# krejciadam/hammock

Hardware: AMD Instinct MI355X
Metric: pairwise BLOSUM62 ShiftedScorer scores/sec (all-vs-all, thresholded neighbour list) (higher is better)
Workload: dtype u8 (8-bit SWAR lanes, host-proven ranges with 16-bit / literal fallbacks; scores are int32-exact)

## Files before the change

### hammock_amd/csrc/hmk_common.cpp

```cpp
#include <atomic>

#include "hmk_ctx.h"
#include "hmk_grid.h"

namespace hmk {

static std::atomic<int> g_test_grid_cap{0};
void set_test_grid_cap(int cap) { g_test_grid_cap.store(cap < 1 ? 0 : cap, std::memory_order_relaxed); }
uint32_t capped_grid(const char *kernel, uint32_t wanted) {
    const int cap = g_test_grid_cap.load(std::memory_order_relaxed);
    if (cap < 1 || wanted <= (uint32_t)cap) return wanted;
    std::fprintf(stderr, "[hmk grid] %s %u -> %d\n", kernel, wanted, cap);
    return (uint32_t)cap;
}

namespace impl {

thread_local std::string g_last_error;

void Switches::read() {
    auto flag = [](const char *name) { return getenv(name) != nullptr; };
    auto num = [](const char *name, int dflt) { const char *v = getenv(name); return v ? atoi(v) : dflt; };
    *this = Switches();
    greedy_timing = flag("HMK_GREEDY_TIMING");
    no_band = flag("HMK_NO_BAND");
    no_rows_kernel = flag("HMK_NO_ROWS_KERNEL");
    key_sort = flag("HMK_NO_KEY_SORT") ? 0 : num("HMK_KEY_SORT_KEYS", 2) == 1 ? 1 : 2;
    no_row_shared = flag("HMK_NO_ROW_SHARED");
    adj_8byte = flag("HMK_ADJ_8BYTE");
    local_literal = flag("HMK_LOCAL_LITERAL");
    local_signed = flag("HMK_LOCAL_SIGNED");
    local_no_pk = flag("HMK_LOCAL_NO_PK");
    multi_replicate = flag("HMK_MULTI_REPLICATE");
    multi_force_copies = flag("HMK_MULTI_FORCE_COPIES");
    if (const char *v = getenv("HMK_SECOND_LOOP")) second_loop = std::strcmp(v, "device") == 0 ? 1 : 2;
    phase1_threads = std::max(0, num("HMK_PHASE1_THREADS", 0));
    phase1_window = std::max(0, num("HMK_PHASE1_WINDOW", 0));
    if (const char *v = getenv("HMK_PHASE1_HOST_BAND")) {
        host_band_rows = std::max(0, atoi(v));
        if (const char *c = std::strchr(v, ',')) host_band_far_t = std::max(0, atoi(c + 1));
    }
    loop_chain = getenv("HMK_LOOP_CHAIN") ? (num("HMK_LOOP_CHAIN", 0) != 0 ? 1 : 0) : -1;
    loop_passes = std::min(8, std::max(0, num("HMK_LOOP_PASSES", 0)));
// ... 218 lines not shown
```

### hammock_amd/csrc/hmk_ctx.h

```cpp
#ifndef HMK_CTX_H
#define HMK_CTX_H
#include <hip/hip_runtime_api.h>

#include <algorithm>
#include <chrono>
#include <condition_variable>
#include <functional>
#include <future>
#include <memory>
#include <cstdio>
#include <cstdlib>
#include <cstring>
#include <map>
#include <mutex>
#include <numeric>
#include <string>
#include <tuple>
#include <thread>
#include <vector>

#include "hmk_internal.h"
#include "hmk_kernels.h"
#include "hmk_sizing.h"

// ... 54 lines not shown
    SB_MERGE_CNT, SB_MERGE_OSTART, SB_MERGE_SCR, SB_MERGE_SCAN,
    SB_LINK_TAB, SB_LINK_OUT,
    SB_SPLIT_SCORES,
    SB_CC_PARENT, SB_CC_SIZE,
    SB_CC_STATE, SB_CC_RUNS,
    SB_ALIGN_SLOT, SB_ALIGN_MEMB,
    SB_N
};

struct Switches {
    bool greedy_timing = false;
    bool no_band = false;
    bool no_rows_kernel = false;
    int key_sort = 2;
    bool no_row_shared = false;
    bool adj_8byte = false;
    bool local_literal = false;
    bool local_signed = false;
    bool local_no_pk = false;
    bool multi_replicate = false;
    bool multi_force_copies = false;
    int second_loop = 0;
    int phase1_threads = 0, phase1_window = 0;
    int host_band_rows = 0, host_band_far_t = 0;
    int loop_chain = -1;
    int loop_passes = 0;
    int precheck = 0;
    int late_buffers_delay_ms = 0;
    int csr_bucket_shift = 0;
    uint64_t edge_guess = 0;
// ... 9 lines not shown
    Tile *d_tiles = nullptr;
};

struct Plan : PlanArrays {
    bool valid = false;
    int X = 0, p = 0, thr = 0;
    uint32_t part = 0, n_parts = 1;
    uint32_t band_rows = 0;
    int64_t band_req = 0;
    int lbmax = 12, lpad = 16;
    bool exact = false;
    bool rows_exact = false;
    bool no_rows_kernel = false;
    int key_sort = 2;
    bool row_shared = true;
    uint32_t *d_keyrun = nullptr;
    uint32_t *d_keytab = nullptr;
    uint32_t cols_per_tile = 16384;
    uint8_t *d_mb = nullptr;
    std::vector<Group> groups;
    hmk_neighbor_stats stats{};
    uint64_t band_pairs = 0;
    uint32_t q0 = 0, q1 = 0, r0 = 0, r1 = 0;
};

struct PlanLocal : PlanArrays {
    bool valid = false;
    uint32_t part = 0, n_parts = 1;
    uint32_t n_tiles = 0;
    uint64_t pairs = 0;
// ... 261 lines not shown
```

### hammock_amd/csrc/hmk_internal.h

```cpp
#ifndef HMK_INTERNAL_H
#define HMK_INTERNAL_H

#include <stdint.h>

#include <functional>
#include <string>
#include <vector>

#include "../../include/hammock_hip.h"

namespace hmk {


enum { PATH_U8 = 0, PATH_U16 = 1, PATH_DIRECT = 2, PATH_ROWS = 3 };

struct TileClass {
    uint8_t la, lb;
    uint8_t nd;
    uint8_t case_b;
    uint8_t x;
    uint8_t path;
    uint8_t nw;
    uint8_t pad;
    int32_t g;
// ... 19 lines not shown
    uint64_t *edges;
    unsigned long long *counts;
    uint64_t cap_per_shard;
    uint32_t n_tiles;
    uint32_t lpad;
    uint32_t symmetric;
    uint32_t row_is_m;
    uint32_t perm_identity;
    uint32_t *deg;
    uint32_t deg_m_offset;
    const uint32_t *keyrun;
    const uint32_t *keytab;
};

constexpr int KEYTAB_DWORDS = 16;
constexpr bool rows_keyed(int x, int d, int cap, bool exact, int g) { return exact && d == 0 && g == 1 && x == 3 && cap == 12; }
constexpr int rows_key_pos(int x, int l, int q) { return l / 2 - 1 + q < x ? x : l / 2 - 1 + q; }

struct Nbr {
    uint32_t m;
    int32_t s;
    uint32_t id() const { return m; }
    int32_t score() const { return s; }
};
struct NbrPacked {
    uint32_t v;
    uint32_t id() const { return v >> 8; }
    int32_t score() const { return (int32_t)(v & 0xFFu); }
};

struct GreedyCand { int32_t c, mn, covered; };
// ... 84 lines not shown
```

### hammock_amd/csrc/hmk_kernels.h

```cpp
#ifndef HMK_KERNELS_H
#define HMK_KERNELS_H

#include <hip/hip_runtime_api.h>
#include <stdint.h>

#include "hmk_internal.h"

namespace hmk {

int swar_rows_per_tile(int lbmax, int nw, bool exact);
int swar_lbmax_for(int lb);

hipError_t launch_neighbors_swar(int lbmax, int nw, bool exact, const NeighborParams &P,
                                 uint32_t tile_base, uint32_t n_tiles, hipStream_t s);
bool rows_kernel_available(int X, int la, int lb, bool exact);
int rows_cap_for(int lb);
int rows_per_tile_rows(int X, int d, int cap, bool exact);
hipError_t launch_neighbors_rows(int X, int d, int cap, bool exact, const NeighborParams &P, uint32_t tile_base,
                                 uint32_t n_tiles, hipStream_t s);
hipError_t warm_neighbors_rows_module();
hipError_t launch_rows_keytab(const uint8_t *res_sorted, uint32_t lpad, uint32_t n, const uint8_t *mb, int case_b, int X, int L,
                              const uint32_t (&cinit)[8], uint32_t *keytab, uint32_t n_groups);
hipError_t launch_neighbors_direct(const NeighborParams &P, uint32_t tile_base, uint32_t n_tiles,
                                   const int32_t *d_matrix, int max_shift, int shift_penalty, int threshold,
                                   hipStream_t s);
hipError_t launch_probe_spin(unsigned long long *when, long long ticks, hipStream_t s);
hipError_t launch_pairs(int scorer, const uint8_t *res32, const uint8_t *len, const int32_t *d_matrix,
                        const uint32_t *pi, const uint32_t *pj, uint64_t n_pairs, uint32_t r0, uint32_t c0,
                        uint32_t width, int a, int b, int32_t *out, int32_t *out_shift, hipStream_t s);

hipError_t launch_neighbors_local(int lbmax, bool enc, bool force_signed, bool force_unpacked, const NeighborParams &P, uint32_t tile_base,
                                  uint32_t n_tiles, const int32_t *d_matrix, int gap_open, int gap_extend, int threshold, hipStream_t s);

hipError_t launch_neighbors_local_literal(const NeighborParams &P, uint32_t tile_base, uint32_t n_tiles, const int32_t *d_matrix,
// ... 96 lines not shown
```

### hammock_amd/csrc/hmk_pass.cpp

```cpp
#include "hmk_ctx.h"

namespace hmk { namespace impl {

static int make_side_streams(hmk_ctx *ctx) {
    constexpr int n_side = hmk_ctx::N_SIDE, MAX_TRIES = 12;
    unsigned long long *when = nullptr;
    HIPCHK(ctx, hipHostMalloc((void **)&when, 64, hipHostMallocDefault));
    auto side_by_side = [&](hipStream_t a, hipStream_t b, bool *yes) -> hipError_t {
        std::memset(when, 0, 64);
        hipError_t e = launch_probe_spin(when, 6000, a);
        if (e == hipSuccess) e = launch_probe_spin(when + 2, 6000, b);
        if (e == hipSuccess) e = hipStreamSynchronize(a);
        if (e == hipSuccess) e = hipStreamSynchronize(b);
        *yes = when[2] < when[1] && when[0] < when[3];
        return e;
    };
    std::vector<hipStream_t> kept, dropped;
    hipError_t e = hipSuccess;
    for (int t = 0; t < MAX_TRIES && (int)kept.size() < n_side && e == hipSuccess; t++) {
        hipStream_t s = nullptr;
        e = hipStreamCreateWithFlags(&s, hipStreamNonBlocking);
        if (e != hipSuccess) break;
        bool ok = true;
        for (size_t k = 0; k < kept.size() && ok && e == hipSuccess; k++) e = side_by_side(kept[k], s, &ok);
// ... 56 lines not shown
    std::vector<const Group *> order;
    for (const Group &g : pl.groups) order.push_back(&g);
    std::stable_sort(order.begin(), order.end(), [](const Group *a, const Group *b) { return a->work > b->work; });
    uint64_t load[hmk_ctx::N_SIDE] = {0};
    for (const Group *gp : order) {
        const Group &g = *gp;
        int least = 0;
        for (int k = 1; k < n_side; k++) if (load[k] < load[least]) least = k;
        load[least] += g.work;
        hipStream_t s = fork ? sides[least] : stream;
        const uint32_t t0 = which == LAUNCH_REST ? g.base + g.band : g.base;
        const uint32_t cnt = which == LAUNCH_ALL ? g.count : which == LAUNCH_BAND ? g.band : g.count - g.band;
        if (g.path == PATH_DIRECT)
            HIPCHK(ctx, launch_neighbors_direct(P, t0, cnt, ctx->d_M.as<int32_t>(), X, p, thr, s));
        else if (g.path == PATH_ROWS)
            HIPCHK(ctx, launch_neighbors_rows(X, g.nw, g.lbk, pl.rows_exact, P, t0, cnt, s));
        else
            HIPCHK(ctx, launch_neighbors_swar(g.lbk, g.nw, pl.exact, P, t0, cnt, s));
    }
    if (fork)
        for (int k = 0; k < n_side; k++) {
            HIPCHK(ctx, hipEventRecord(ctx->ev_join[k], sides[k]));
            HIPCHK(ctx, hipStreamWaitEvent(stream, ctx->ev_join[k], 0));
        }
    return HMK_OK;
}

bool local_enc(const hmk_ctx *ctx, int gap_open, int gap_extend) {
    return ctx->min_m >= -31 && ctx->max_m <= 31 && gap_open >= -31 && gap_extend >= -31 && gap_open <= 0 && gap_extend <= 0;
}

// ... 165 lines not shown
```

### hammock_amd/csrc/hmk_plan.cpp

```cpp
#include "hmk_ctx.h"

namespace hmk { namespace impl {

template <class T, class Cmp>
void parallel_stable_sort(std::vector<T> &v, Cmp before) {
    const size_t n = v.size();
    const unsigned hw = usable_cpus();
    size_t runs = 1;
    while (runs < 8 && runs < (hw ? hw : 1u) && n / (2 * runs) >= 32768) runs *= 2;
    if (runs == 1) { std::stable_sort(v.begin(), v.end(), before); return; }
    std::vector<size_t> cut(runs + 1);
    for (size_t r = 0; r <= runs; r++) cut[r] = n * r / runs;
    {
        std::vector<std::thread> pool;
        for (size_t r = 1; r < runs; r++) pool.emplace_back([&, r] { std::stable_sort(v.begin() + (long)cut[r], v.begin() + (long)cut[r + 1], before); });
        std::stable_sort(v.begin(), v.begin() + (long)cut[1], before);
        for (std::thread &th : pool) th.join();
    }
    std::vector<T> other(n);
    std::vector<T> *from = &v, *to = &other;
    for (size_t width = 1; width < runs; width *= 2) {
        std::vector<std::thread> pool;
        for (size_t r = 0; r < runs; r += 2 * width) {
            auto job = [&, r] {
// ... 20 lines not shown
    for (int side = 0; side < 2; side++) {
        uint32_t *b = bucket[side];
        std::fill(b, b + HMK_MAX_LEN + 2, 0u);
        for (uint32_t k = lo[side]; k < hi[side]; k++) b[ctx->len[k] + 1]++;
        b[0] = side ? a1 - a0 : 0u;
        for (int l = 0; l <= HMK_MAX_LEN; l++) b[l + 1] += b[l];
        Buckets fill;
        std::memcpy(fill, b, sizeof(fill));
        for (uint32_t k = lo[side]; k < hi[side]; k++) perm[fill[ctx->len[k]]++] = k;
    }
}

using GroupKey = std::tuple<int, int, int>;
struct KernelChoice { bool rows; int lbk; uint32_t R; GroupKey key; };

KernelChoice choose_kernel(const TileClass &tc, int X, bool use_rows, bool rows_exact, bool exact) {
    const int la = tc.la, lb = tc.lb;
    KernelChoice k;
    k.rows = use_rows && tc.path == PATH_U8 && la >= lb && (rows_exact || rows_kernel_available(X, la, lb, false));
    k.lbk = k.rows ? (rows_exact ? lb : rows_cap_for(lb)) : exact ? 12 : swar_lbmax_for(lb);
    k.R = k.rows ? (uint32_t)rows_per_tile_rows(X, la - lb, k.lbk, rows_exact)
                 : tc.path == PATH_DIRECT ? 16u : (uint32_t)swar_rows_per_tile(k.lbk, tc.nw, exact);
    k.key = k.rows ? GroupKey((int)PATH_ROWS, la - lb, k.lbk)
                   : GroupKey((int)tc.path, tc.path == PATH_DIRECT ? 0 : (int)tc.nw, tc.path == PATH_DIRECT ? 0 : k.lbk);
    return k;
}

uint32_t add_class(std::vector<TileClass> &classes, hmk_neighbor_stats &S, const TileClass &tc, bool rows) {
    classes.push_back(tc);
    if (tc.path == PATH_U8) S.classes_u8++;
    else if (tc.path == PATH_U16) S.classes_u16++;
    else S.classes_direct++;
    if (rows) S.classes_rows++;
    return (uint32_t)classes.size() - 1;
}

// ... 190 lines not shown
        c.path = u16 ? PATH_U16 : PATH_U8;
        c.g = (int32_t)g;
        const int lpd = u16 ? 2 : 4, bits = u16 ? 16 : 8;
        const int ndw = (nd + lpd - 1) / lpd;
        c.nw = (uint8_t)ndw;
        for (int t = 0; t < nd; t++) c.cinit[t / lpd] |= (uint32_t)ci[t] << ((t % lpd) * bits);
    }
    *out = c;
}

int build_plan(hmk_ctx *ctx, int X, int p, int thr, uint32_t part, uint32_t n_parts, int64_t band_rows, bool key_sort_ok) {
    Plan &pl = ctx->plan;
    const int want_keys = key_sort_ok ? ctx->sw.key_sort : 0;
    if (pl.valid && pl.X == X && pl.p == p && pl.thr == thr && pl.part == part && pl.n_parts == n_parts &&
        (band_rows < 0 || pl.band_req == band_rows) && pl.no_rows_kernel == ctx->sw.no_rows_kernel && pl.key_sort == want_keys &&
        pl.row_shared == !ctx->sw.no_row_shared)
        return HMK_OK;
    free_plan(pl);
    if (band_rows < 0) band_rows = 0;
    const int64_t band_req = band_rows;
    const bool plan_timing = ctx->sw.greedy_timing;
    const auto plan_t0 = std::chrono::steady_clock::now();
    auto plan_lap = [&](const char *what) {
        if (plan_timing)
            fprintf(stderr, "[hmk plan] %s at %.2f ms\n", what,
                    std::chrono::duration<double, std::milli>(std::chrono::steady_clock::now() - plan_t0).count());
    };
    const uint32_t n = ctx->n;
    if (n == 0) return fail(ctx, HMK_ERR_NO_SEQUENCES, "no sequences set (hmk_set_sequences)");
    if (X < 0) return fail(ctx, HMK_ERR_BAD_ARG, "max_shift must be >= 0");
    if (n_parts == 0 || part >= n_parts) return fail(ctx, HMK_ERR_BAD_ARG, "part must be < n_parts");
// ... 74 lines not shown
    pl.no_rows_kernel = ctx->sw.no_rows_kernel;
    pl.exact = false;
    pl.rows_exact = false;
    if (use_rows && ctx->min_len == ctx->max_len) {
        TileClass t1;
        classify(ctx, ctx->min_len, ctx->min_len, X, p, thr, &t1);
        pl.rows_exact = (t1.path == PATH_U8 || (refine && all_rows_fit)) && rows_kernel_available(X, ctx->min_len, ctx->min_len, true);
    }
    if (!use_rows && ctx->min_len == 12 && ctx->max_len == 12 && X == 3) {
        TileClass t12;
        classify(ctx, 12, 12, X, p, thr, &t12);
        pl.exact = t12.path == PATH_U8 && t12.nw == 2;
    }
    pl.key_sort = want_keys;
    pl.row_shared = !ctx->sw.no_row_shared;
    std::vector<uint32_t> keyrun;
    const int L1 = ctx->min_len;
    const bool key_sorted = pl.key_sort > 0 && pl.rows_exact && !(refine && !all_rows_fit) &&
                            rows_keyed(X, 0, L1, true, rows_per_tile_rows(X, 0, L1, true) / 8) && n >= 2;
    if (key_sorted) {
        const int k0 = rows_key_pos(X, L1, 0), k1 = rows_key_pos(X, L1, 1);
        auto key_of = [&](uint32_t k) { return (uint32_t)ctx->res[ctx->off[k] + k0] * HMK_ALPHABET + ctx->res[ctx->off[k] + k1]; };
        const uint32_t b0 = band_end[L1], b1 = bucket[L1 + 1];
        std::vector<uint32_t> cnt(HMK_ALPHABET * HMK_ALPHABET + 1, 0u), sorted(perm.begin() + b0, perm.begin() + b1);
        for (uint32_t q = b0; q < b1; q++) cnt[key_of(perm[q]) + 1]++;
        for (int v = 0; v < HMK_ALPHABET * HMK_ALPHABET; v++) cnt[v + 1] += cnt[v];
        for (uint32_t q = b0; q < b1; q++) sorted[cnt[key_of(perm[q])]++] = perm[q];
        std::copy(sorted.begin(), sorted.end(), perm.begin() + b0);
        keyrun.resize(2 * (size_t)n);
        uint32_t r0 = 0, r01 = 0;
        for (uint32_t q = 0; q < n; q++) {
            const uint32_t k = perm[q], c0 = ctx->res[ctx->off[k] + k0], c1 = ctx->res[ctx->off[k] + k1];
            if (q > 0) {
                const uint32_t kp = perm[q - 1];
                const bool same0 = ctx->res[ctx->off[kp] + k0] == c0;
                r0 += same0 ? 0u : 1u;
                r01 += (pl.key_sort == 2 && same0 && ctx->res[ctx->off[kp] + k1] == c1) ? 0u : 1u;
            }
            keyrun[2 * (size_t)q] = r0 << 5 | c0;
            keyrun[2 * (size_t)q + 1] = r01 << 5 | c1;
        }
    }
    const uint64_t tile_rows = pl.rows_exact ? (uint64_t)rows_per_tile_rows(X, 0, ctx->min_len, true) : use_rows ? 16 : 6;
    const uint64_t row_groups = (uint64_t)n / tile_rows / n_parts + 1;
    pl.cols_per_tile = 65536;
    while (pl.cols_per_tile > 16384 && row_groups * ((uint64_t)n / (2 * pl.cols_per_tile) + 1) < 8 * 1792)
        pl.cols_per_tile /= 2;
    while (pl.cols_per_tile > 4096 && ((uint64_t)n / tile_rows + 1) * ((uint64_t)n / (2 * pl.cols_per_tile) + 1) < 4096)
        pl.cols_per_tile /= 2;

    std::vector<TileClass> classes;
    std::map<GroupKey, std::vector<Tile>> grouped;
    hmk_neighbor_stats &S = pl.stats;
    S = hmk_neighbor_stats{};
    S.symmetric = ctx->symmetric;
    uint64_t row_chunk_counter = 0;
    for (int la = 1; la <= HMK_MAX_LEN; la++) {
        const uint32_t rb = bucket[la], re = bucket[la + 1];
        if (rb == re) continue;
        for (int lb = 1; lb <= HMK_MAX_LEN; lb++) {
            const uint32_t cb = bucket[lb], ce = bucket[lb + 1];
            if (cb == ce) continue;
// ... 10 lines not shown
                if (refine && tc0.path != PATH_U8 && limit >= 0) {
                    const uint32_t lim = (uint32_t)std::min<long long>(limit, BCAP - 1);
                    split = all_rows_fit ? re
                                         : (uint32_t)(std::upper_bound(bound_sorted.begin() + rb, bound_sorted.begin() + re, lim) -
                                                      bound_sorted.begin());
                    if (split > rb) {
                        TileClass t8;
                        classify(ctx, la, lb, X, p, thr, &t8, lim);
                        if (t8.path == PATH_U8) ranges.push_back(Range{rb, split, t8});
                        else split = rb;
                    }
                }
                if (split < re) ranges.push_back(Range{split, re, tc0});
            }
            for (const Range &rg : ranges) {
                const KernelChoice k = choose_kernel(rg.tc, X, use_rows, pl.rows_exact, pl.exact);
                const uint32_t cls = add_class(classes, S, rg.tc, k.rows);
                std::vector<Tile> &dst = grouped[k.key];
                const bool tri = same && ctx->symmetric;
                for (uint32_t r0 = rg.lo; r0 < rg.hi; r0 += k.R) {
                    if ((row_chunk_counter++ % n_parts) != part) continue;
                    Band band{r0 < band_end[la], band_end[lb], 0};
                    S.pairs_scored += emit_tiles(dst, cls, r0, std::min(k.R, rg.hi - r0), tri ? r0 + 1 : cb, ce, pl.cols_per_tile, true,
                                                 tri ? 1u : same ? 2u : 0u, &band);
                    pl.band_pairs += band.pairs;
                }
            }
        }
    }
    plan_lap("classes and tiles");
    std::vector<Tile> tiles = order_groups(grouped, classes, X, pl.groups);
// ... 194 lines not shown
```

### hammock_amd/csrc/k_neighbors_rows.h

```cpp
#ifndef HMK_NEIGHBORS_ROWS_H
#define HMK_NEIGHBORS_ROWS_H
#include "hmk_device.h"

namespace hmk {

constexpr int ROWS_STAGE_CAPFORM = 320, ROWS_STAGE_EXACT = 640, ROWS_STAGE_SHORT = 1024;
constexpr int ROWS_INLOOP_MAXCELLS = 45;
constexpr int rows_cells(int x, int cap) { return cap * (2 * x + 1) - x * (x + 1); }
constexpr bool rows_inloop(int x, int cap) { return rows_cells(x, cap) > ROWS_INLOOP_MAXCELLS; }
constexpr bool rows_inloop_shape(int x, int d, int cap, bool exact) { return (exact && d > 0) || rows_inloop(x, cap); }
constexpr int rows_stage(int x, int d, int cap, bool exact) {
    return !exact ? ROWS_STAGE_CAPFORM : rows_inloop_shape(x, d, cap, exact) ? ROWS_STAGE_EXACT : ROWS_STAGE_SHORT;
}
constexpr int rows_groups(int x, int , int cap, bool exact) {
    return !exact ? 2 : rows_inloop(x, cap) ? 1 : 2;
}
constexpr bool rows_two_ended(int x, int d, int cap, bool exact, int g) { return exact && !rows_inloop_shape(x, d, cap, exact) && g == 2; }

template <typename T>
__device__ __forceinline__ T rows_table_read(uint32_t addr) {
    return *reinterpret_cast<const volatile HMK_LDS T *>((uintptr_t)addr);
}
constexpr int rows_waves(int nd, int cap, int lds_bytes, bool exact) {
    const int v = cap + 2 * nd + 36 + (exact ? 0 : 6);
// ... 475 lines not shown
#undef HMK_FLUSH_ST
#undef HMK_FLUSH_ST_00
#undef HMK_FLUSH_ST_01
#undef HMK_FLUSH_ST_10
#undef HMK_FLUSH_ST_11
    asm volatile("" ::: "memory");
    drain_end();
    }
}

template <class F, int... Is>
__device__ __forceinline__ void rows_for_each_group(std::integer_sequence<int, Is...>, F &&f) {
    (f(std::integral_constant<int, Is>{}), ...);
}

template <int X, int D, int CAP, bool EXACT_LB, int G, int MODE>
__device__ __forceinline__ void rows_tile(const NeighborParams &P, const uint32_t tile_base, uint8_t *smem) {
    using S = RowsShape<X, D, CAP, EXACT_LB, G>;
    constexpr int ND = S::ND, NI = S::NI, NEND = S::NEND, TAB_BYTES = S::TAB_BYTES;
    constexpr int R = 8 * G;
    constexpr int STAGE_CAP = rows_stage(X, D, CAP, EXACT_LB);
    constexpr int LDS_BYTES = TAB_BYTES + 576 + R * 32 + 4 * STAGE_CAP * 4;
    static_assert(LDS_BYTES == rows_lds_bytes(X, D, CAP, EXACT_LB, G), "rows_lds_bytes must match the LDS map");
    uint8_t *tab = smem;
    uint8_t *mb = smem + TAB_BYTES;
    uint8_t *rowres = mb + 576;
    uint32_t *stage_all = reinterpret_cast<uint32_t *>(rowres + R * 32);

    const Tile T = P.tiles[tile_base + blockIdx.x];
    const TileClass *Cp = P.classes + T.cls;
    const int la = Cp->la;
    int lbs = EXACT_LB ? CAP : (int)Cp->lb;
    const bool case_b = Cp->case_b != 0;
    const int tid = threadIdx.x;
    HMK_LDS uint32_t *stage = (HMK_LDS uint32_t *)stage_all + __builtin_amdgcn_readfirstlane(tid >> 6) * STAGE_CAP;

    constexpr bool KEYED = rows_keyed(X, D, CAP, EXACT_LB, G);
    const bool keyed = KEYED && P.keyrun != nullptr;
    const bool row_shared = keyed && (T.row_shared & 1u) != 0;

    build_begin();
    const uint32_t tab_addr = lds_addr(tab);
    for (int e = tid; e < 576; e += 256) mb[e] = P.mb[e];
    for (int e = tid; e < R * 32; e += 256) {
        const int r = e >> 5, k = e & 31;
        uint8_t v = 0;
        if ((uint32_t)r < T.nrows && (uint32_t)k < P.lpad) v = P.res_sorted[(size_t)(T.row0 + r) * P.lpad + k];
        rowres[e] = v;
    }
    __syncthreads();
    for (int e = tid; e < G * (NI + NEND) * 24 * 2; e += 256) {
        const int h = e & 1, ic = e >> 1;
        const int gi = ic / 24, c = ic - gi * 24;
        const int g = gi / (NI + NEND), k = gi - g * (NI + NEND);
        int i = k < NI ? k : la - 1 - (k - NI);
        const int dst = k < NI ? S::pos_addr(g, k) : S::end_addr(g, k - NI);
        if constexpr (KEYED)
            if (row_shared && k == S::key_pos(0) && h == 1) i = S::key_pos(1);
        uint32_t v = 0;
        if (i >= 0 && i < la) {
#pragma unroll
            for (int q = 0; q < 4; q++) {
                const int r = 8 * g + 4 * h + q;
                if ((uint32_t)r < T.nrows) {
                    const int a = rowres[r * 32 + i];
                    v |= (uint32_t)(case_b ? mb[c * 24 + a] : mb[a * 24 + c]) << (q * 8);
                }
            }
        }
        *reinterpret_cast<uint32_t *>(tab + dst + c * 8 + h * 4) = v;
    }
    __syncthreads();
    build_end();
// ... 8 lines not shown
    const uint32_t col_end = T.col0 + T.ncols;
    const uint32_t n_batches = (T.ncols + 255) / 256;
    const bool interior = T.diag == 0 && T.ncols % 256 == 0;
    const bool prio = true;

    const uint8_t *const res_sorted = P.res_sorted;
    const uint32_t lpad_s = P.lpad;

    constexpr bool INLOOP = rows_inloop_shape(X, D, CAP, EXACT_LB);
    constexpr bool DEFER = EXACT_LB && !INLOOP;
    const uint64_t ka64 = (uint64_t)(uintptr_t)__builtin_amdgcn_kernarg_segment_ptr();
    const uint32_t ka_lo = (uint32_t)ka64, ka_hi = (uint32_t)(ka64 >> 32);
    uint32_t acc[G];
#pragma unroll
    for (int g = 0; g < G; g++) acc[g] = 0;
    static_assert(!KEYED || (G == 1 && 2 * ND <= KEYTAB_DWORDS), "key table entry; one row group per tile");
    static_assert(!KEYED || (S::body_reads(3, false) == 58 && S::body_reads(1, false) == 65 && S::body_reads(0, false) == 72), "ordinary bodies");
    static_assert(!KEYED || (S::body_reads(3, true) == 54 && S::body_reads(1, true) == 60 && S::body_reads(0, true) == 66), "row-shared bodies");
    const uint32_t wave = __builtin_amdgcn_readfirstlane(tid >> 6);
    const uint32_t *kt_tile = nullptr, *kr_wave = nullptr;
    if (keyed) {
        kt_tile = P.keytab + (size_t)(T.row0 >> 3) * (2 * 24 * KEYTAB_DWORDS);
        kr_wave = P.keyrun + 2 * (size_t)(T.col0 + wave * 64);
    }
    auto key_entry = [](const uint32_t *e, uint32_t (&k0)[ND], uint32_t (&k1)[ND]) {
#pragma unroll
        for (int u = 0; u + 1 < ND; u += 2) {
            const u32x4 a = rows_const_load<u32x4>(e + 2 * u);
            k0[u] = a.x; k1[u] = a.y; k0[u + 1] = a.z; k1[u + 1] = a.w;
        }
        if constexpr (ND & 1) {
// ... 14 lines not shown
                const uint32_t last = min(63u, col_end - 1u - wc0);
                ra = rows_const_load<u32x2>(kr_wave);
                const u32x2 rb = rows_const_load<u32x2>(kr_wave + 2 * last);
                if (ra.x == rb.x) kmode = ra.y == rb.y ? 3 : 1;
            }
        }
        uint32_t off[CAP], toff[S::NT];
        S::offsets_of(words, tw, tab_addr, tab_addr, off, toff);
        const bool look = !DEFER || (bt & 3u) == 3u || bt + 1 == n_batches;

        auto one_group = [&](auto gt) {
            constexpr int g = decltype(gt)::value;
            if ((uint32_t)(8 * g) >= T.nrows) return;
            uint32_t W0[ND], W1[ND];
            if constexpr (KEYED) {
                uint32_t ks0[ND], ks1[ND];
                if (kmode == 3) {
                    uint32_t kb0[ND], kb1[ND];
                    key_entry(kt_tile + (ra.x & 31u) * KEYTAB_DWORDS, ks0, ks1);
                    key_entry(kt_tile + (24 + (ra.y & 31u)) * KEYTAB_DWORDS, kb0, kb1);
#pragma unroll
                    for (int u = 0; u < ND; u++) { ks0[u] += kb0[u]; ks1[u] += kb1[u]; }
                    read_phase_begin(prio);
                    if (row_shared) S::template accumulate<g, 3, true>(off, toff, lbs, ks0, ks1, W0, W1);
                    else S::template accumulate<g, 3>(off, toff, lbs, ks0, ks1, W0, W1);
                } else if (kmode == 1) {
                    key_entry(kt_tile + (ra.x & 31u) * KEYTAB_DWORDS, ks0, ks1);
#pragma unroll
                    for (int u = 0; u < ND; u++) asm volatile("" : "+s"(ks0[u]), "+s"(ks1[u]));
                    read_phase_begin(prio);
                    if (row_shared) S::template accumulate<g, 1, true>(off, toff, lbs, ks0, ks1, W0, W1);
                    else S::template accumulate<g, 1>(off, toff, lbs, ks0, ks1, W0, W1);
                } else {
                    read_phase_begin(prio);
                    if (row_shared) S::template accumulate<g, 0, true>(off, toff, lbs, ci, ci, W0, W1);
                    else S::template accumulate<g>(off, toff, lbs, ci, ci, W0, W1);
                }
            } else {
                read_phase_begin(prio);
                S::template accumulate<g>(off, toff, lbs, ci, ci, W0, W1);
            }
            read_phase_end(prio);
// ... 82 lines not shown
    return m;
}
constexpr int rows_lens_waves(int x, int d, int capb) {
    const int lds = rows_lens_lds(x, d, capb);
    int w = rows_waves(2 * x + d + 1, capb, lds, false);
    for (int lb = rows_lens_first(capb); lb <= capb; lb++)
        if (rows_lens_has(x, d, capb, lb) && rows_waves(2 * x + d + 1, lb, lds, true) < w) w = rows_waves(2 * x + d + 1, lb, lds, true);
    return w;
}
template <int X, int D, int CAPB, int MODE, int LB>
__device__ __forceinline__ void rows_lens_pick(const NeighborParams &P, const uint32_t tile_base, uint8_t *smem, int lb) {
    if constexpr (LB > CAPB) {
        rows_tile<X, D, CAPB, false, 2, MODE>(P, tile_base, smem);
    } else {
        if constexpr (rows_lens_has(X, D, CAPB, LB)) {
            if (lb == LB) { rows_tile<X, D, LB, true, 2, MODE>(P, tile_base, smem); return; }
        }
        rows_lens_pick<X, D, CAPB, MODE, LB + 1>(P, tile_base, smem, lb);
    }
}
template <int X, int D, int CAPB, int MODE>
__global__ void __launch_bounds__(256, rows_lens_waves(X, D, CAPB))
k_neighbors_rows_lens(const NeighborParams P, const uint32_t tile_base) {
    __shared__ __attribute__((aligned(16))) uint8_t smem[rows_lens_lds(X, D, CAPB)];
    const int lb = (int)P.classes[P.tiles[tile_base + blockIdx.x].cls].lb;
    rows_lens_pick<X, D, CAPB, MODE, rows_lens_first(CAPB)>(P, tile_base, smem, lb);
}


}
#endif
// ... 1 lines not shown
```

### hammock_amd/csrc/k_neighbors_rows.hip

```cpp
#include "k_rows_shapes.h"

namespace hmk {

int rows_cap_for(int lb) { return lb <= 12 ? 12 : lb <= 16 ? 16 : lb <= 20 ? 20 : 0; }

namespace {
int rows_part_of(int X, int d, int cap, bool exact) {
    if (exact) {
#define HMK_F(PV, XV, L) if (X == XV && d == 0 && cap == L) return PV;
        HMK_ROWS_EXACT_LIST(HMK_F)
#undef HMK_F
        return -1;
    }
#define HMK_C(PV, XV, DV, CAPV) if (X == XV && d == DV && cap == CAPV) return PV;
    HMK_ROWS_CAP_LIST(HMK_C)
#undef HMK_C
    return -1;
}
}

int rows_per_tile_rows(int X, int d, int cap, bool exact) {
    if (rows_part_of(X, d, cap, exact) < 0) return 0;
    return 8 * rows_groups(X, d, cap, exact);
}

bool rows_kernel_available(int X, int la, int lb, bool exact) {
    if (la < lb || lb < 2 * X || X < 1) return false;
    return rows_part_of(X, la - lb, exact ? lb : rows_cap_for(lb), exact) >= 0;
}

hipError_t launch_neighbors_rows(int X, int d, int cap, bool exact, const NeighborParams &P, uint32_t tile_base,
                                 uint32_t n_tiles, hipStream_t s) {
    if (n_tiles == 0) return hipSuccess;
    switch (rows_part_of(X, d, cap, exact)) {
#define HMK_P(p) case p: return launch_rows_part_##p(X, d, cap, exact, P, tile_base, n_tiles, s);
        HMK_P(0) HMK_P(1) HMK_P(2) HMK_P(3) HMK_P(4) HMK_P(5) HMK_P(6) HMK_P(7) HMK_P(8) HMK_P(9) HMK_P(10) HMK_P(11) HMK_P(12)
#undef HMK_P
    }
    return hipErrorInvalidValue;
}

hipError_t warm_neighbors_rows_module() { return warm_rows_part_0(); }

struct KeytabInit { uint32_t w[8]; };
__global__ void __launch_bounds__(256) k_rows_keytab(const uint8_t *__restrict__ res_sorted, uint32_t lpad, uint32_t n,
                                                     const uint8_t *__restrict__ mb, int case_b, int X, int L, const KeytabInit cinit,
                                                     uint32_t *__restrict__ keytab, uint32_t n_groups) {
    const uint64_t e = (uint64_t)blockIdx.x * 256 + threadIdx.x;
    if (e >= (uint64_t)n_groups * 2 * HMK_ALPHABET * KEYTAB_DWORDS) return;
    const int d = (int)(e % KEYTAB_DWORDS), c = (int)(e / KEYTAB_DWORDS % HMK_ALPHABET), q = (int)(e / (KEYTAB_DWORDS * HMK_ALPHABET) % 2);
// ... 29 lines not shown
```

### hammock_amd/csrc/k_rows_part.hip

```cpp
#include "k_rows_shapes.h"

#ifndef HMK_ROWS_PART
#error "compile with -DHMK_ROWS_PART=<part>"
#endif

namespace hmk {

namespace {
template <bool MINE, int X, int D, int CAP, bool EXACT_LB>
struct RowsLaunch {
    static hipError_t go(const NeighborParams &, uint32_t, uint32_t, hipStream_t) { return hipErrorInvalidValue; }
};
template <int X, int D, int CAP, bool EXACT_LB>
struct RowsLaunch<true, X, D, CAP, EXACT_LB> {
    static hipError_t go(const NeighborParams &P, uint32_t tile_base, uint32_t n_tiles, hipStream_t s) {
        return launch_rows_t<X, D, CAP, EXACT_LB>(P, tile_base, n_tiles, s);
    }
};
}

#define HMK_CAT2(a, b) a##b
#define HMK_CAT(a, b) HMK_CAT2(a, b)

hipError_t HMK_CAT(launch_rows_part_, HMK_ROWS_PART)(int X, int d, int cap, bool exact, const NeighborParams &P, uint32_t tile_base,
                                                     uint32_t n_tiles, hipStream_t s) {
    if (exact) {
#define HMK_F(PV, XV, L) \
    if (PV == HMK_ROWS_PART && X == XV && d == 0 && cap == L) return RowsLaunch<PV == HMK_ROWS_PART, XV, 0, L, true>::go(P, tile_base, n_tiles, s);
        HMK_ROWS_EXACT_LIST(HMK_F)
#undef HMK_F
        return hipErrorInvalidValue;
    }
#define HMK_C(PV, XV, DV, CAPV) \
    if (PV == HMK_ROWS_PART && X == XV && d == DV && cap == CAPV) return RowsLaunch<PV == HMK_ROWS_PART, XV, DV, CAPV, false>::go(P, tile_base, n_tiles, s);
    HMK_ROWS_CAP_LIST(HMK_C)
#undef HMK_C
    return hipErrorInvalidValue;
}

#if HMK_ROWS_PART == 0
hipError_t warm_rows_part_0() {
    hipFuncAttributes a;
    return hipFuncGetAttributes(&a, reinterpret_cast<const void *>(&k_neighbors_rows<3, 0, 12, true, rows_groups(3, 0, 12, true), EDGES_PLAIN>));
}
#endif

}
```

### hammock_amd/csrc/k_rows_shapes.h

```cpp
#ifndef HMK_ROWS_SHAPES_H
#define HMK_ROWS_SHAPES_H
#include "k_neighbors_rows.h"

namespace hmk {

template <int X, int D, int CAP, bool EXACT_LB>
static hipError_t launch_rows_t(const NeighborParams &P, uint32_t tile_base, uint32_t n_tiles, hipStream_t s) {
    constexpr int G = rows_groups(X, D, CAP, EXACT_LB);
    if constexpr (!EXACT_LB && (X == 2 || X == 3)) {
        static_assert(G == 2, "the planner gives the capacity groups 16 rows per tile");
        if (P.deg) hipLaunchKernelGGL((k_neighbors_rows_lens<X, D, CAP, EDGES_COUNT>), dim3(n_tiles), dim3(256), 0, s, P, tile_base);
        else hipLaunchKernelGGL((k_neighbors_rows_lens<X, D, CAP, EDGES_PLAIN>), dim3(n_tiles), dim3(256), 0, s, P, tile_base);
        return hipGetLastError();
    } else {
        if (P.deg)
            hipLaunchKernelGGL((k_neighbors_rows<X, D, CAP, EXACT_LB, G, EDGES_COUNT>), dim3(n_tiles), dim3(256), 0, s, P, tile_base);
        else
            hipLaunchKernelGGL((k_neighbors_rows<X, D, CAP, EXACT_LB, G, EDGES_PLAIN>), dim3(n_tiles), dim3(256), 0, s, P, tile_base);
        return hipGetLastError();
    }
}

#define HMK_ROWS_EXACT_LIST(F) \
    F(0, 3, 10) F(0, 3, 11) F(0, 3, 12) F(0, 3, 13) \
// ... 5 lines not shown
    C(8, 3, 8, 12) C(9, 3, 9, 12) C(9, 3, 10, 12) C(9, 3, 11, 12) C(9, 3, 12, 12) C(9, 3, 13, 12) \
    C(2, 3, 0, 16) C(2, 3, 1, 16) C(2, 3, 2, 16) C(2, 3, 3, 16) C(10, 3, 4, 16) C(10, 3, 5, 16) C(10, 3, 6, 16) C(10, 3, 7, 16) \
    C(10, 3, 0, 20) C(10, 3, 1, 20) C(10, 3, 2, 20) C(10, 3, 3, 20) \
    C(3, 1, 0, 12) C(3, 1, 1, 12) C(3, 1, 2, 12) C(3, 1, 3, 12) C(3, 1, 4, 12) \
    C(11, 2, 0, 12) C(11, 2, 1, 12) C(11, 2, 2, 12) C(11, 2, 3, 12) C(12, 2, 4, 12) C(12, 2, 5, 12) C(12, 2, 6, 12) C(12, 2, 7, 12) \
    C(3, 2, 0, 16) C(3, 2, 1, 16) C(3, 2, 2, 16) C(3, 2, 3, 16) \
    C(4, 4, 0, 12) C(4, 4, 1, 12) C(4, 4, 2, 12) C(4, 4, 3, 12) C(4, 4, 4, 12) C(4, 4, 5, 12) C(4, 4, 6, 12) C(4, 4, 7, 12) \
    C(4, 4, 8, 12) \
    C(5, 4, 0, 16) C(5, 4, 1, 16) C(5, 4, 2, 16) C(5, 4, 3, 16) C(5, 4, 4, 16) C(5, 4, 5, 16) C(5, 4, 6, 16) C(5, 4, 7, 16) \
    C(5, 4, 0, 20) C(5, 4, 1, 20) C(5, 4, 2, 20) C(5, 4, 3, 20) \
    C(6, 5, 0, 12) C(6, 5, 1, 12) C(6, 5, 2, 12) \
    C(6, 5, 0, 16) C(6, 5, 1, 16) C(6, 5, 2, 16) C(6, 5, 3, 16) C(6, 5, 4, 16) \
    C(6, 5, 0, 20) C(6, 5, 1, 20) C(6, 5, 2, 20) C(6, 5, 3, 20) C(6, 5, 4, 20)

#define HMK_ROWS_PART_DECL(p) \
    hipError_t launch_rows_part_##p(int X, int d, int cap, bool exact, const NeighborParams &P, uint32_t tile_base, uint32_t n_tiles, hipStream_t s);
HMK_ROWS_PART_DECL(0) HMK_ROWS_PART_DECL(1) HMK_ROWS_PART_DECL(2) HMK_ROWS_PART_DECL(3)
HMK_ROWS_PART_DECL(4) HMK_ROWS_PART_DECL(5) HMK_ROWS_PART_DECL(6) HMK_ROWS_PART_DECL(7)
HMK_ROWS_PART_DECL(8) HMK_ROWS_PART_DECL(9) HMK_ROWS_PART_DECL(10) HMK_ROWS_PART_DECL(11) HMK_ROWS_PART_DECL(12)
#undef HMK_ROWS_PART_DECL
hipError_t warm_rows_part_0();

}
#endif
```

Before: 2442 billion.

## Let keyed rows kernel handle two row groups per tile when tiles are plentiful

Extends the key-sorted exact rows kernel (X=3, d=0, cap 12) so one tile can cover two 8-row groups, each with its own key-table slice and row-shared bit. The planner turns this on by default when the estimated tile count stays above a threshold, and the HMK_KEY_ROW_PAIRS override can force it on or off. The aim is to amortise each tile's column-table build and LDS staging over twice as many rows. In exchange there are fewer tiles, which can hurt load balance and occupancy, and the kernel carries more registers for two accumulators. The length-dispatch kernel turns key forms off so it keeps its old behaviour.

```diff
diff --git a/hammock_amd/csrc/hmk_common.cpp b/hammock_amd/csrc/hmk_common.cpp
--- a/hammock_amd/csrc/hmk_common.cpp
+++ b/hammock_amd/csrc/hmk_common.cpp
@@ -27,6 +27,7 @@
     no_rows_kernel = flag("HMK_NO_ROWS_KERNEL");
     key_sort = flag("HMK_NO_KEY_SORT") ? 0 : num("HMK_KEY_SORT_KEYS", 2) == 1 ? 1 : 2;
     no_row_shared = flag("HMK_NO_ROW_SHARED");
+    key_row_pairs = getenv("HMK_KEY_ROW_PAIRS") ? (num("HMK_KEY_ROW_PAIRS", 0) != 0 ? 1 : 0) : -1;
     adj_8byte = flag("HMK_ADJ_8BYTE");
     local_literal = flag("HMK_LOCAL_LITERAL");
     local_signed = flag("HMK_LOCAL_SIGNED");
diff --git a/hammock_amd/csrc/hmk_ctx.h b/hammock_amd/csrc/hmk_ctx.h
--- a/hammock_amd/csrc/hmk_ctx.h
+++ b/hammock_amd/csrc/hmk_ctx.h
@@ -92,6 +92,7 @@
     bool no_rows_kernel = false;
     int key_sort = 2;
     bool no_row_shared = false;
+    int key_row_pairs = -1;
     bool adj_8byte = false;
     bool local_literal = false;
     bool local_signed = false;
@@ -131,6 +132,8 @@
     bool no_rows_kernel = false;
     int key_sort = 2;
     bool row_shared = true;
+    int key_row_pairs = -1;
+    bool key_pairs = false;
     uint32_t *d_keyrun = nullptr;
     uint32_t *d_keytab = nullptr;
     uint32_t cols_per_tile = 16384;
diff --git a/hammock_amd/csrc/hmk_internal.h b/hammock_amd/csrc/hmk_internal.h
--- a/hammock_amd/csrc/hmk_internal.h
+++ b/hammock_amd/csrc/hmk_internal.h
@@ -57,7 +57,8 @@
 };
 
 constexpr int KEYTAB_DWORDS = 16;
-constexpr bool rows_keyed(int x, int d, int cap, bool exact, int g) { return exact && d == 0 && g == 1 && x == 3 && cap == 12; }
+constexpr int ROWS_KEY_PAIR_GROUPS = 2;
+constexpr bool rows_keyed(int x, int d, int cap, bool exact, int g) { return exact && d == 0 && (g == 1 || g == ROWS_KEY_PAIR_GROUPS) && x == 3 && cap == 12; }
 constexpr int rows_key_pos(int x, int l, int q) { return l / 2 - 1 + q < x ? x : l / 2 - 1 + q; }
 
 struct Nbr {
diff --git a/hammock_amd/csrc/hmk_kernels.h b/hammock_amd/csrc/hmk_kernels.h
--- a/hammock_amd/csrc/hmk_kernels.h
+++ b/hammock_amd/csrc/hmk_kernels.h
@@ -15,9 +15,9 @@
                                  uint32_t tile_base, uint32_t n_tiles, hipStream_t s);
 bool rows_kernel_available(int X, int la, int lb, bool exact);
 int rows_cap_for(int lb);
-int rows_per_tile_rows(int X, int d, int cap, bool exact);
+int rows_per_tile_rows(int X, int d, int cap, bool exact, bool key_pairs = false);
 hipError_t launch_neighbors_rows(int X, int d, int cap, bool exact, const NeighborParams &P, uint32_t tile_base,
-                                 uint32_t n_tiles, hipStream_t s);
+                                 uint32_t n_tiles, bool key_pairs, hipStream_t s);
 hipError_t warm_neighbors_rows_module();
 hipError_t launch_rows_keytab(const uint8_t *res_sorted, uint32_t lpad, uint32_t n, const uint8_t *mb, int case_b, int X, int L,
                               const uint32_t (&cinit)[8], uint32_t *keytab, uint32_t n_groups);
diff --git a/hammock_amd/csrc/hmk_pass.cpp b/hammock_amd/csrc/hmk_pass.cpp
--- a/hammock_amd/csrc/hmk_pass.cpp
+++ b/hammock_amd/csrc/hmk_pass.cpp
@@ -94,7 +94,7 @@
         if (g.path == PATH_DIRECT)
             HIPCHK(ctx, launch_neighbors_direct(P, t0, cnt, ctx->d_M.as<int32_t>(), X, p, thr, s));
         else if (g.path == PATH_ROWS)
-            HIPCHK(ctx, launch_neighbors_rows(X, g.nw, g.lbk, pl.rows_exact, P, t0, cnt, s));
+            HIPCHK(ctx, launch_neighbors_rows(X, g.nw, g.lbk, pl.rows_exact, P, t0, cnt, pl.key_pairs, s));
         else
             HIPCHK(ctx, launch_neighbors_swar(g.lbk, g.nw, pl.exact, P, t0, cnt, s));
     }
diff --git a/hammock_amd/csrc/hmk_plan.cpp b/hammock_amd/csrc/hmk_plan.cpp
--- a/hammock_amd/csrc/hmk_plan.cpp
+++ b/hammock_amd/csrc/hmk_plan.cpp
@@ -58,12 +58,12 @@
 using GroupKey = std::tuple<int, int, int>;
 struct KernelChoice { bool rows; int lbk; uint32_t R; GroupKey key; };
 
-KernelChoice choose_kernel(const TileClass &tc, int X, bool use_rows, bool rows_exact, bool exact) {
+KernelChoice choose_kernel(const TileClass &tc, int X, bool use_rows, bool rows_exact, bool exact, bool key_pairs = false) {
     const int la = tc.la, lb = tc.lb;
     KernelChoice k;
     k.rows = use_rows && tc.path == PATH_U8 && la >= lb && (rows_exact || rows_kernel_available(X, la, lb, false));
     k.lbk = k.rows ? (rows_exact ? lb : rows_cap_for(lb)) : exact ? 12 : swar_lbmax_for(lb);
-    k.R = k.rows ? (uint32_t)rows_per_tile_rows(X, la - lb, k.lbk, rows_exact)
+    k.R = k.rows ? (uint32_t)rows_per_tile_rows(X, la - lb, k.lbk, rows_exact, key_pairs)
                  : tc.path == PATH_DIRECT ? 16u : (uint32_t)swar_rows_per_tile(k.lbk, tc.nw, exact);
     k.key = k.rows ? GroupKey((int)PATH_ROWS, la - lb, k.lbk)
                    : GroupKey((int)tc.path, tc.path == PATH_DIRECT ? 0 : (int)tc.nw, tc.path == PATH_DIRECT ? 0 : k.lbk);
@@ -284,7 +284,7 @@
     const int want_keys = key_sort_ok ? ctx->sw.key_sort : 0;
     if (pl.valid && pl.X == X && pl.p == p && pl.thr == thr && pl.part == part && pl.n_parts == n_parts &&
         (band_rows < 0 || pl.band_req == band_rows) && pl.no_rows_kernel == ctx->sw.no_rows_kernel && pl.key_sort == want_keys &&
-        pl.row_shared == !ctx->sw.no_row_shared)
+        pl.row_shared == !ctx->sw.no_row_shared && pl.key_row_pairs == ctx->sw.key_row_pairs)
         return HMK_OK;
     free_plan(pl);
     if (band_rows < 0) band_rows = 0;
@@ -389,6 +389,7 @@
     }
     pl.key_sort = want_keys;
     pl.row_shared = !ctx->sw.no_row_shared;
+    pl.key_row_pairs = ctx->sw.key_row_pairs;
     std::vector<uint32_t> keyrun;
     const int L1 = ctx->min_len;
     const bool key_sorted = pl.key_sort > 0 && pl.rows_exact && !(refine && !all_rows_fit) &&
@@ -416,11 +417,18 @@
             keyrun[2 * (size_t)q + 1] = r01 << 5 | c1;
         }
     }
-    const uint64_t tile_rows = pl.rows_exact ? (uint64_t)rows_per_tile_rows(X, 0, ctx->min_len, true) : use_rows ? 16 : 6;
-    const uint64_t row_groups = (uint64_t)n / tile_rows / n_parts + 1;
-    pl.cols_per_tile = 65536;
-    while (pl.cols_per_tile > 16384 && row_groups * ((uint64_t)n / (2 * pl.cols_per_tile) + 1) < 8 * 1792)
-        pl.cols_per_tile /= 2;
+    auto tiles_about = [&](uint64_t tile_rows, uint32_t cols) { return ((uint64_t)n / tile_rows / n_parts + 1) * ((uint64_t)n / (2 * cols) + 1); };
+    auto cols_for = [&](uint64_t tile_rows) {
+        uint32_t cols = 65536;
+        while (cols > 16384 && tiles_about(tile_rows, cols) < 8 * 1792) cols /= 2;
+        return cols;
+    };
+    constexpr uint64_t KEY_PAIR_MIN_TILES = 6 * 2048;
+    const uint64_t paired_rows = key_sorted ? (uint64_t)rows_per_tile_rows(X, 0, L1, true, true) : 0;
+    pl.key_pairs = paired_rows != 0 && (ctx->sw.key_row_pairs >= 0 ? ctx->sw.key_row_pairs == 1
+                                                                   : tiles_about(paired_rows, cols_for(paired_rows)) >= KEY_PAIR_MIN_TILES);
+    const uint64_t tile_rows = pl.key_pairs ? paired_rows : pl.rows_exact ? (uint64_t)rows_per_tile_rows(X, 0, ctx->min_len, true) : use_rows ? 16 : 6;
+    pl.cols_per_tile = cols_for(tile_rows);
     while (pl.cols_per_tile > 4096 && ((uint64_t)n / tile_rows + 1) * ((uint64_t)n / (2 * pl.cols_per_tile) + 1) < 4096)
         pl.cols_per_tile /= 2;
 
@@ -461,7 +469,7 @@
                 if (split < re) ranges.push_back(Range{split, re, tc0});
             }
             for (const Range &rg : ranges) {
-                const KernelChoice k = choose_kernel(rg.tc, X, use_rows, pl.rows_exact, pl.exact);
+                const KernelChoice k = choose_kernel(rg.tc, X, use_rows, pl.rows_exact, pl.exact, pl.key_pairs);
                 const uint32_t cls = add_class(classes, S, rg.tc, k.rows);
                 std::vector<Tile> &dst = grouped[k.key];
                 const bool tri = same && ctx->symmetric;
diff --git a/hammock_amd/csrc/k_neighbors_rows.h b/hammock_amd/csrc/k_neighbors_rows.h
--- a/hammock_amd/csrc/k_neighbors_rows.h
+++ b/hammock_amd/csrc/k_neighbors_rows.h
@@ -513,7 +513,7 @@
     (f(std::integral_constant<int, Is>{}), ...);
 }
 
-template <int X, int D, int CAP, bool EXACT_LB, int G, int MODE>
+template <int X, int D, int CAP, bool EXACT_LB, int G, int MODE, bool KEY_FORMS = true>
 __device__ __forceinline__ void rows_tile(const NeighborParams &P, const uint32_t tile_base, uint8_t *smem) {
     using S = RowsShape<X, D, CAP, EXACT_LB, G>;
     constexpr int ND = S::ND, NI = S::NI, NEND = S::NEND, TAB_BYTES = S::TAB_BYTES;
@@ -534,9 +534,10 @@
     const int tid = threadIdx.x;
     HMK_LDS uint32_t *stage = (HMK_LDS uint32_t *)stage_all + __builtin_amdgcn_readfirstlane(tid >> 6) * STAGE_CAP;
 
-    constexpr bool KEYED = rows_keyed(X, D, CAP, EXACT_LB, G);
+    constexpr bool KEYED = KEY_FORMS && rows_keyed(X, D, CAP, EXACT_LB, G);
     const bool keyed = KEYED && P.keyrun != nullptr;
-    const bool row_shared = keyed && (T.row_shared & 1u) != 0;
+    const bool rs_first = keyed && (T.row_shared & 1u) != 0;
+    const uint32_t rs_groups = keyed ? T.row_shared : 0u;
 
     build_begin();
     const uint32_t tab_addr = lds_addr(tab);
@@ -555,7 +556,7 @@
         int i = k < NI ? k : la - 1 - (k - NI);
         const int dst = k < NI ? S::pos_addr(g, k) : S::end_addr(g, k - NI);
         if constexpr (KEYED)
-            if (row_shared && k == S::key_pos(0) && h == 1) i = S::key_pos(1);
+            if ((G == 1 ? rs_first : ((rs_groups >> g) & 1u) != 0) && k == S::key_pos(0) && h == 1) i = S::key_pos(1);
         uint32_t v = 0;
         if (i >= 0 && i < la) {
 #pragma unroll
@@ -594,7 +595,7 @@
     uint32_t acc[G];
 #pragma unroll
     for (int g = 0; g < G; g++) acc[g] = 0;
-    static_assert(!KEYED || (G == 1 && 2 * ND <= KEYTAB_DWORDS), "key table entry; one row group per tile");
+    static_assert(!KEYED || (G <= 2 && 2 * ND <= KEYTAB_DWORDS), "key table entry; at most two row groups per tile");
     static_assert(!KEYED || (S::body_reads(3, false) == 58 && S::body_reads(1, false) == 65 && S::body_reads(0, false) == 72), "ordinary bodies");
     static_assert(!KEYED || (S::body_reads(3, true) == 54 && S::body_reads(1, true) == 60 && S::body_reads(0, true) == 66), "row-shared bodies");
     const uint32_t wave = __builtin_amdgcn_readfirstlane(tid >> 6);
@@ -639,18 +640,20 @@
             if ((uint32_t)(8 * g) >= T.nrows) return;
             uint32_t W0[ND], W1[ND];
             if constexpr (KEYED) {
+                const uint32_t *const kt_group = kt_tile + (size_t)g * (2 * 24 * KEYTAB_DWORDS);
+                const bool row_shared = G == 1 ? rs_first : (rs_groups & (1u << g)) != 0;
                 uint32_t ks0[ND], ks1[ND];
                 if (kmode == 3) {
                     uint32_t kb0[ND], kb1[ND];
-                    key_entry(kt_tile + (ra.x & 31u) * KEYTAB_DWORDS, ks0, ks1);
-                    key_entry(kt_tile + (24 + (ra.y & 31u)) * KEYTAB_DWORDS, kb0, kb1);
+                    key_entry(kt_group + (ra.x & 31u) * KEYTAB_DWORDS, ks0, ks1);
+                    key_entry(kt_group + (24 + (ra.y & 31u)) * KEYTAB_DWORDS, kb0, kb1);
 #pragma unroll
                     for (int u = 0; u < ND; u++) { ks0[u] += kb0[u]; ks1[u] += kb1[u]; }
                     read_phase_begin(prio);
                     if (row_shared) S::template accumulate<g, 3, true>(off, toff, lbs, ks0, ks1, W0, W1);
                     else S::template accumulate<g, 3>(off, toff, lbs, ks0, ks1, W0, W1);
                 } else if (kmode == 1) {
-                    key_entry(kt_tile + (ra.x & 31u) * KEYTAB_DWORDS, ks0, ks1);
+                    key_entry(kt_group + (ra.x & 31u) * KEYTAB_DWORDS, ks0, ks1);
 #pragma unroll
                     for (int u = 0; u < ND; u++) asm volatile("" : "+s"(ks0[u]), "+s"(ks1[u]));
                     read_phase_begin(prio);
@@ -763,7 +766,7 @@
         rows_tile<X, D, CAPB, false, 2, MODE>(P, tile_base, smem);
     } else {
         if constexpr (rows_lens_has(X, D, CAPB, LB)) {
-            if (lb == LB) { rows_tile<X, D, LB, true, 2, MODE>(P, tile_base, smem); return; }
+            if (lb == LB) { rows_tile<X, D, LB, true, 2, MODE, false>(P, tile_base, smem); return; }
         }
         rows_lens_pick<X, D, CAPB, MODE, LB + 1>(P, tile_base, smem, lb);
     }
diff --git a/hammock_amd/csrc/k_neighbors_rows.hip b/hammock_amd/csrc/k_neighbors_rows.hip
--- a/hammock_amd/csrc/k_neighbors_rows.hip
+++ b/hammock_amd/csrc/k_neighbors_rows.hip
@@ -19,8 +19,9 @@
 }
 }
 
-int rows_per_tile_rows(int X, int d, int cap, bool exact) {
+int rows_per_tile_rows(int X, int d, int cap, bool exact, bool key_pairs) {
     if (rows_part_of(X, d, cap, exact) < 0) return 0;
+    if (key_pairs) return rows_keyed(X, d, cap, exact, ROWS_KEY_PAIR_GROUPS) ? 8 * ROWS_KEY_PAIR_GROUPS : 0;
     return 8 * rows_groups(X, d, cap, exact);
 }
 
@@ -30,10 +31,10 @@
 }
 
 hipError_t launch_neighbors_rows(int X, int d, int cap, bool exact, const NeighborParams &P, uint32_t tile_base,
-                                 uint32_t n_tiles, hipStream_t s) {
+                                 uint32_t n_tiles, bool key_pairs, hipStream_t s) {
     if (n_tiles == 0) return hipSuccess;
     switch (rows_part_of(X, d, cap, exact)) {
-#define HMK_P(p) case p: return launch_rows_part_##p(X, d, cap, exact, P, tile_base, n_tiles, s);
+#define HMK_P(p) case p: return launch_rows_part_##p(X, d, cap, exact, P, tile_base, n_tiles, key_pairs, s);
         HMK_P(0) HMK_P(1) HMK_P(2) HMK_P(3) HMK_P(4) HMK_P(5) HMK_P(6) HMK_P(7) HMK_P(8) HMK_P(9) HMK_P(10) HMK_P(11) HMK_P(12)
 #undef HMK_P
     }
diff --git a/hammock_amd/csrc/k_rows_part.hip b/hammock_amd/csrc/k_rows_part.hip
--- a/hammock_amd/csrc/k_rows_part.hip
+++ b/hammock_amd/csrc/k_rows_part.hip
@@ -9,12 +9,12 @@
 namespace {
 template <bool MINE, int X, int D, int CAP, bool EXACT_LB>
 struct RowsLaunch {
-    static hipError_t go(const NeighborParams &, uint32_t, uint32_t, hipStream_t) { return hipErrorInvalidValue; }
+    static hipError_t go(const NeighborParams &, uint32_t, uint32_t, bool, hipStream_t) { return hipErrorInvalidValue; }
 };
 template <int X, int D, int CAP, bool EXACT_LB>
 struct RowsLaunch<true, X, D, CAP, EXACT_LB> {
-    static hipError_t go(const NeighborParams &P, uint32_t tile_base, uint32_t n_tiles, hipStream_t s) {
-        return launch_rows_t<X, D, CAP, EXACT_LB>(P, tile_base, n_tiles, s);
+    static hipError_t go(const NeighborParams &P, uint32_t tile_base, uint32_t n_tiles, bool key_pairs, hipStream_t s) {
+        return launch_rows_t<X, D, CAP, EXACT_LB>(P, tile_base, n_tiles, key_pairs, s);
     }
 };
 }
@@ -23,16 +23,16 @@
 #define HMK_CAT(a, b) HMK_CAT2(a, b)
 
 hipError_t HMK_CAT(launch_rows_part_, HMK_ROWS_PART)(int X, int d, int cap, bool exact, const NeighborParams &P, uint32_t tile_base,
-                                                     uint32_t n_tiles, hipStream_t s) {
+                                                     uint32_t n_tiles, bool key_pairs, hipStream_t s) {
     if (exact) {
 #define HMK_F(PV, XV, L) \
-    if (PV == HMK_ROWS_PART && X == XV && d == 0 && cap == L) return RowsLaunch<PV == HMK_ROWS_PART, XV, 0, L, true>::go(P, tile_base, n_tiles, s);
+    if (PV == HMK_ROWS_PART && X == XV && d == 0 && cap == L) return RowsLaunch<PV == HMK_ROWS_PART, XV, 0, L, true>::go(P, tile_base, n_tiles, key_pairs, s);
         HMK_ROWS_EXACT_LIST(HMK_F)
 #undef HMK_F
         return hipErrorInvalidValue;
     }
 #define HMK_C(PV, XV, DV, CAPV) \
-    if (PV == HMK_ROWS_PART && X == XV && d == DV && cap == CAPV) return RowsLaunch<PV == HMK_ROWS_PART, XV, DV, CAPV, false>::go(P, tile_base, n_tiles, s);
+    if (PV == HMK_ROWS_PART && X == XV && d == DV && cap == CAPV) return RowsLaunch<PV == HMK_ROWS_PART, XV, DV, CAPV, false>::go(P, tile_base, n_tiles, key_pairs, s);
     HMK_ROWS_CAP_LIST(HMK_C)
 #undef HMK_C
     return hipErrorInvalidValue;
diff --git a/hammock_amd/csrc/k_rows_shapes.h b/hammock_amd/csrc/k_rows_shapes.h
--- a/hammock_amd/csrc/k_rows_shapes.h
+++ b/hammock_amd/csrc/k_rows_shapes.h
@@ -5,8 +5,17 @@
 namespace hmk {
 
 template <int X, int D, int CAP, bool EXACT_LB>
-static hipError_t launch_rows_t(const NeighborParams &P, uint32_t tile_base, uint32_t n_tiles, hipStream_t s) {
+static hipError_t launch_rows_t(const NeighborParams &P, uint32_t tile_base, uint32_t n_tiles, bool key_pairs, hipStream_t s) {
     constexpr int G = rows_groups(X, D, CAP, EXACT_LB);
+    if constexpr (rows_keyed(X, D, CAP, EXACT_LB, ROWS_KEY_PAIR_GROUPS) && G != ROWS_KEY_PAIR_GROUPS) {
+        if (key_pairs) {
+            if (!P.keyrun || P.deg) return hipErrorInvalidValue;
+            hipLaunchKernelGGL((k_neighbors_rows<X, D, CAP, EXACT_LB, ROWS_KEY_PAIR_GROUPS, EDGES_PLAIN>), dim3(n_tiles), dim3(256), 0, s, P, tile_base);
+            return hipGetLastError();
+        }
+    } else if (key_pairs) {
+        return hipErrorInvalidValue;
+    }
     if constexpr (!EXACT_LB && (X == 2 || X == 3)) {
         static_assert(G == 2, "the planner gives the capacity groups 16 rows per tile");
         if (P.deg) hipLaunchKernelGGL((k_neighbors_rows_lens<X, D, CAP, EDGES_COUNT>), dim3(n_tiles), dim3(256), 0, s, P, tile_base);
@@ -43,7 +52,7 @@
     C(6, 5, 0, 20) C(6, 5, 1, 20) C(6, 5, 2, 20) C(6, 5, 3, 20) C(6, 5, 4, 20)
 
 #define HMK_ROWS_PART_DECL(p) \
-    hipError_t launch_rows_part_##p(int X, int d, int cap, bool exact, const NeighborParams &P, uint32_t tile_base, uint32_t n_tiles, hipStream_t s);
+    hipError_t launch_rows_part_##p(int X, int d, int cap, bool exact, const NeighborParams &P, uint32_t tile_base, uint32_t n_tiles, bool key_pairs, hipStream_t s);
 HMK_ROWS_PART_DECL(0) HMK_ROWS_PART_DECL(1) HMK_ROWS_PART_DECL(2) HMK_ROWS_PART_DECL(3)
 HMK_ROWS_PART_DECL(4) HMK_ROWS_PART_DECL(5) HMK_ROWS_PART_DECL(6) HMK_ROWS_PART_DECL(7)
 HMK_ROWS_PART_DECL(8) HMK_ROWS_PART_DECL(9) HMK_ROWS_PART_DECL(10) HMK_ROWS_PART_DECL(11) HMK_ROWS_PART_DECL(12)
```

After: 2498 billion, median of 6. +2.3%, better.
